# jiaqianjing/kubedl

Hardware: AMD Instinct MI355X
Metric: Job launch delay (s) + steps/sec, PyTorchJob ResNet-50 at 1/2/4/8 MI355X (higher is better)
Workload: dtype bf16

## Files before the change

csrc/bindings.cpp:

```cpp
#include <map>
#include <mutex>
#include <cstring>
#include <torch/extension.h>
#include <ATen/hip/HIPContext.h>
#include <ATen/hip/impl/HIPGuardImplMasqueradingAsCUDA.h>
#include <ATen/hip/impl/HIPStreamMasqueradingAsCUDA.h>

#include "bn_fin.h"
#include "kdl_api.h"

namespace {

int dtype_code(const at::Tensor& t) {
  if (t.scalar_type() == at::kBFloat16) return 1;
  if (t.scalar_type() == at::kFloat) return 0;
  TORCH_CHECK(false, "kubedl_amd: unsupported dtype ", t.scalar_type());
  return -1;
}

hipStream_t cur_stream() { return c10::hip::getCurrentHIPStreamMasqueradingAsCUDA().stream(); }

void check_hip(hipError_t e, const char* what) {
  TORCH_CHECK(e == hipSuccess, "kubedl_amd: ", what, " failed: ", hipGetErrorString(e));
}
// ... 1363 lines not shown
  const int64_t rows_in = stride > 1 ? (M / (Hout * Wout)) * Hin * Win : M;
  need_bf16(G, M * N, "conv1x1_wgrad G");
  need_bf16(A, rows_in * K, "conv1x1_wgrad A");
  need_opt_f32(pro_coef, 2 * K, "pro_coef");
  const int64_t slabs =
      kdl::conv1x1_wgrad_splits(static_cast<int>(M), static_cast<int>(N), static_cast<int>(K), solo);
  TORCH_CHECK(dw32.is_cuda() && dw32.scalar_type() == at::kFloat && dw32.is_contiguous() &&
                  dw32.numel() >= slabs * N * K,
              "conv1x1_wgrad: dw32 must be fp32 contiguous with conv1x1_wgrad_splits(M, N, K) * N * K elements");
  if (dW.has_value() && dW->defined())
    TORCH_CHECK(dW->is_cuda() && dW->is_contiguous() && dW->numel() == N * K && dW->scalar_type() == at::kBFloat16,
                "conv1x1_wgrad: dW bf16 contiguous [N, K]");
  const c10::hip::HIPGuardMasqueradingAsCUDA guard(G.device());
  check_hip(kdl::conv1x1_wgrad(G.data_ptr(), A.data_ptr(), opt_fptr(pro_coef), dw32.data_ptr<float>(),
                               dW.has_value() && dW->defined() ? dW->data_ptr() : nullptr, static_cast<float>(scale),
                               static_cast<int>(M), static_cast<int>(N), static_cast<int>(K), static_cast<int>(Hout),
                               static_cast<int>(Wout), static_cast<int>(Hin), static_cast<int>(Win),
                               static_cast<int>(stride), cur_stream(), bw.x, bw.coef, solo),
            "conv1x1_wgrad");
}

int64_t conv1x1_gram_floats(int64_t M, int64_t K) {
  return static_cast<int64_t>(kdl::conv1x1_gram_splits(static_cast<int>(M), static_cast<int>(K))) * (K * K + K);
}

void conv1x1_gram(const at::Tensor& X, const at::Tensor& pro, at::Tensor ws, int64_t M, int64_t K) {
  need_bf16(X, M * K, "conv1x1_gram X");
  need_opt_f32(pro, 2 * K, "conv1x1_gram pro");
  need_opt_f32(ws, conv1x1_gram_floats(M, K), "conv1x1_gram ws");
  const c10::hip::HIPGuardMasqueradingAsCUDA guard(X.device());
  check_hip(kdl::conv1x1_gram(X.data_ptr(), pro.data_ptr<float>(), ws.data_ptr<float>(), static_cast<int>(M),
                              static_cast<int>(K), cur_stream()),
            "conv1x1_gram");
}

void gram_fold(const at::Tensor& Gm, const at::Tensor& QS, const at::Tensor& W, const at::Tensor& bcoef, at::Tensor out,
               int64_t N, int64_t K) {
  need_opt_f32(Gm, N * K, "gram_fold G");
  need_opt_f32(QS, K * K + K, "gram_fold Q|s");
  need_opt_f32(bcoef, 3 * N, "gram_fold bcoef");
  need_bf16(W, N * K, "gram_fold W");
  need_bf16(out, N * K, "gram_fold out");
  const c10::hip::HIPGuardMasqueradingAsCUDA guard(W.device());
  check_hip(kdl::gram_fold(Gm.data_ptr<float>(), QS.data_ptr<float>(), W.data_ptr(), bcoef.data_ptr<float>(),
                           static_cast<int>(N), static_cast<int>(K), out.data_ptr(), cur_stream()),
            "gram_fold");
}

void slab_reduce_f32(at::Tensor slabs, int64_t nk, int64_t nsplit) {
  TORCH_CHECK(nk % 4 == 0 && nsplit >= 1, "slab_reduce_f32: nk % 4 == 0");
  need_opt_f32(slabs, nk * nsplit, "slab_reduce_f32 slabs");
  const c10::hip::HIPGuardMasqueradingAsCUDA guard(slabs.device());
  check_hip(kdl::wgrad_slab_reduce(slabs.data_ptr<float>(), nk, static_cast<int>(nsplit), 1.0f, nullptr,
                                   cur_stream()),
            "slab_reduce_f32");
}

void conv3x3_wgrad(const at::Tensor& G, const at::Tensor& A, const c10::optional<at::Tensor>& pro_coef,
                   at::Tensor dw32, const c10::optional<at::Tensor>& dW, double scale, int64_t Nb, int64_t H,
                   int64_t Wd, int64_t Cin, int64_t Cout, int64_t stride) {
  TORCH_CHECK(Cin % 64 == 0 && Cout % 64 == 0 && Nb > 0 && stride >= 1, "conv3x3_wgrad: need Cin, Cout % 64 == 0");
  const int64_t Ho = (H - 1) / stride + 1, Wo = (Wd - 1) / stride + 1, M = Nb * Ho * Wo, K = 9 * Cin;
  need_bf16(G, M * Cout, "conv3x3_wgrad G");
  need_bf16(A, Nb * H * Wd * Cin, "conv3x3_wgrad A");
  need_opt_f32(pro_coef, 2 * Cin, "pro_coef");
  const int64_t slabs = kdl::conv1x1_wgrad_splits(static_cast<int>(M), static_cast<int>(Cout), static_cast<int>(K));
// ... 245 lines not shown
  m.def("gemm_dgrad_relu", &gemm_dgrad_relu, "(dz W) * [y > 0] and its column sums (bf16): data gradient through a ReLU + bias gradient, one launch");
  m.def("relu_bwd_dbias", &relu_bwd_dbias, "ReLU backward (mask from output) + bias gradient (deterministic; bf16 or fp32)",
        py::arg("dy"), py::arg("y"), py::arg("db_bf16") = false);
  m.def("head_bce_fwd", &head_bce_fwd, "1-wide logit layer + sigmoid BCE: (logit, dlogit, per-block loss sums)");
  m.def("head_bce_bwd", &head_bce_bwd,
        "logit layer backward: (dx, dw, db, per-block dw partials, per-block db partials[, dbx: relu_x])",
        py::arg("x"), py::arg("w"), py::arg("dlogit"), py::arg("scale"), py::arg("gscale"), py::arg("relu_x") = false);
  m.def("embed_gather", &embed_gather, "embedding row gather into a [B, ld] activation");
  m.def("segment_reduce", &segment_reduce, "sorted segment sum of gradient rows", py::arg("rows"), py::arg("F"),
        py::arg("col0"), py::arg("D"), py::arg("order"), py::arg("seg"), py::arg("ucount") = py::none(),
        py::arg("out_rows") = py::none(), py::arg("out") = py::none());
  m.def("a2a_route", &a2a_route, "fixed-capacity exchange: per-owner send blocks + header + rslot of unique ids");
  m.def("a2a_owner_update", &a2a_owner_update, "owner Adagrad update of a fixed exchange without de-duplication",
        py::arg("grads"), py::arg("local"), py::arg("cap"), py::arg("W"), py::arg("slotmap"), py::arg("call"),
        py::arg("table"), py::arg("accum"), py::arg("lr"), py::arg("eps"), py::arg("scale"),
        py::arg("stamped") = false);
  m.def("a2a_serve", &a2a_serve, "owner side of the fixed exchange: requested rows + local row ids (+ the owner "
        "update's slot stamps)",
        py::arg("table"), py::arg("req"), py::arg("n_own"), py::arg("rows_bf16") = false,
        py::arg("slotmap") = py::none(), py::arg("call") = 0, py::arg("cap") = 0, py::arg("W") = 0);
  m.def("embed_gather_cast", &embed_gather_cast,
        "fused one-owner pull: bf16(table[uniq[inv]]) into the tower input (+ tail: dense columns, zero pad)",
        py::arg("table"), py::arg("uniq"), py::arg("inv"), py::arg("F"), py::arg("out"), py::arg("col0"),
        py::arg("dense") = py::none(), py::arg("tail") = 0);
  m.def("segment_adagrad", &segment_adagrad, "segment sum + fused sparse Adagrad on owned rows");
  m.def("dedup_table_slots", &dedup_table_slots, "hash-table slots dedup_csr needs for n ids");
  m.def("segment_reduce_adagrad", &segment_reduce_adagrad,
        "one-owner sync-free push: per-id gradient sums (segment_reduce) applied by Adagrad in the same launch");
  m.def("csr_from_inverse_only", &csr_from_inverse_only, "CSR (seg, order) of a dedup_csr inverse, positions ascending per id");
  m.def("dedup_csr", &dedup_csr, "sync-free id de-duplication (uniq/inv/count on the device) + optional CSR of the inverse");
  m.def("conv1x1_gemm", &conv1x1_gemm, "1x1 conv / dgrad as MFMA GEMM with fused BN prologue/epilogue");
  m.def("set_stem_drop", &kdl::set_stem_drop, "timing-only: skip the stem kernel's MFMAs (1), epilogue (2), input (4)");
  m.def("conv1x1_gram_floats", &conv1x1_gram_floats, "workspace floats of conv1x1_gram(M, K)");
  m.def("conv1x1_gram", &conv1x1_gram, "Q = a^T a | s = 1^T a of a = relu(X*scale+shift) (fp32, into ws[:K*K+K])");
  m.def("gram_fold", &gram_fold, "dW = diag(k) G + diag(c1) W Q + c0 s^T -> bf16 (BN-backward weight gradient, dc never stored)");
  m.def("slab_reduce_f32", &slab_reduce_f32, "fixed-order fp32 sum of slabs into the first");
  m.def("bn_bwd_pro_arm", &bn_bwd_pro_arm, "fuse this BN's backward apply (input x, workspace ws) into the next conv1x1_gemm's A (or conv1x1_wgrad's G) staging; optional write-through tensor");
  m.def("bn_fin_arm", &bn_fin_arm, "fold the BN finalize of this workspace (C channels, M elements) into the next conv GEMM launch");
  m.def("bn_fin_desc", &bn_fin_desc, "write a BN layer's finalize descriptor into its workspace tail");
  m.def("stem7x7_wgrad_bn", &stem7x7_wgrad_bn, "stem weight gradient with the stem BN+ReLU+max-pool backward folded in");
  m.def("stem7x7_wgrad", &stem7x7_wgrad, "ResNet stem 7x7/s2/p3 conv weight gradient -> [64][224] bf16 (stem K order)");
  m.def("stem7x7_wgrad_slabs", [](int64_t nb, int64_t h, int64_t w) {
          return kdl::stem7x7_wgrad_slabs(static_cast<int>(nb), static_cast<int>(h), static_cast<int>(w)); },
        "fp32 slab count of stem7x7_wgrad's workspace", py::arg("nb"), py::arg("h") = 224, py::arg("w") = 224);
  m.def("head_splits", &head_splits, "K splits (fc forward, dfeat) of the classifier head kernels");
  m.def("head_lpad", [](int64_t L) { return kdl::head_lpad(static_cast<int>(L)); }, "row pitch of the head's dl");
  m.def("head_forward", &head_forward, "classifier head forward: mean pool + fc (MFMA) + softmax CE + dlogits");
  m.def("head_backward", &head_backward, "classifier head backward: dfeat, dW, db (MFMA) + mean loss");
  m.def("stem7x7_fwd", &stem7x7_fwd, "ResNet stem 7x7/s2/p3 conv (224 -> 112, 3 -> 64 channels) with BN statistics epilogue");
  m.def("conv3x3_s2_dgrad", &conv3x3_s2_dgrad,
        "stride-2 3x3 pad-1 conv data gradient: four sub-pixel class GEMMs, PLAIN or MASKX epilogue",
        py::arg("dy"), py::arg("ball"), py::arg("dx"), py::arg("Nb"), py::arg("Hd"), py::arg("Wd"), py::arg("Cd"),
        py::arg("N"), py::arg("epi"), py::arg("acc"), py::arg("ex"), py::arg("emean"), py::arg("ecoef"),
        py::arg("Hx") = 0, py::arg("Wx") = 0);
  m.def("bn_res_pro_arm", &bn_res_pro_arm, "next forward conv1x1_gemm applies relu(A*scale+shift+res), written through + mask");
  m.def("conv3x3_aout_arm", &conv3x3_aout_arm, "next prologue conv3x3_gemm also writes relu(B(x)) here (56x56 halo)");
  m.def("conv3x3_gemm", &conv3x3_gemm, "3x3 pad-1 conv (fwd or stride-1 dgrad) as implicit MFMA GEMM with fused BN prologue/epilogue");
  m.def("conv1x1_wgrad", &conv1x1_wgrad, "1x1 conv weight gradient (split-M MFMA into fp32 slabs, fixed-order reduce + bf16 cast); solo: no side stream shares the GPU (more splits)",
        py::arg("G"), py::arg("A"), py::arg("pro_coef"), py::arg("dw32"), py::arg("dW"), py::arg("scale"), py::arg("M"),
        py::arg("N"), py::arg("K"), py::arg("Hout"), py::arg("Wout"), py::arg("Hin"), py::arg("Win"), py::arg("stride"),
        py::arg("solo") = false);
  m.def("conv3x3_wgrad", &conv3x3_wgrad, "3x3 pad-1 conv weight gradient (implicit GEMM, split-M slabs)");
  m.def("conv3x3_wgrad_slabs", &conv3x3_wgrad_slabs, "fp32 [Cout, 9 Cin] slabs conv3x3_wgrad may write (its fastest path)");
  m.def("set_wgrad_big", &kdl::set_wgrad_big, "256x256 weight-gradient tiles: 0 off, 1 3x3 only, 2 3x3 + 1x1");
  m.def("conv1x1_wgrad_splits", &conv1x1_wgrad_splits, "M splits (slab count) of conv1x1_wgrad", py::arg("M"),
        py::arg("N"), py::arg("K"), py::arg("solo") = false);
// ... 12 lines not shown
```

csrc/conv1x1.hip:

```cpp
#include <cstdlib>
#include <type_traits>

#include "common.h"
#include "gemm_epi.h"
#include "kdl_api.h"
#include "tune.h"

namespace kdl {
namespace {

using namespace gemm;

constexpr int kThreads = 256;
constexpr int BK = 64;
__host__ __device__ constexpr int bwd_kmax(int bn) { return bn >= 128 ? 512 : 2048; }

enum { PRO_NONE = 0, PRO_FWD = 1, PRO_BWD = 2, PRO_RES = 5, PRO_RES2 = 6 };

template <int BM, int BN, int MINB, int PRO, int GATHER, int EPI, int KBK = BK>
__global__ __launch_bounds__(kThreads, MINB) void gemm1x1_kernel(GemmParams p, int GM, int tiles_m, int tiles_n) {
  static_assert((PRO != PRO_BWD && PRO != PRO_RES && PRO != PRO_RES2) || GATHER == G_DENSE,
                "the two-input prologues read dense rows");
  constexpr bool TWO_IN = PRO == PRO_BWD || PRO == PRO_RES || PRO == PRO_RES2;
  constexpr int LDK = KBK + 8;
// ... 723 lines not shown
  const int a = wgrad_splits(M, N, K, false), b = wgrad_splits(M, N, K, false, true);
  const int c = solo ? wgrad_splits(M, N, K, false, false, true) : 0;
  return a > b ? (a > c ? a : c) : (b > c ? b : c);
}

void set_wgrad_big(int mode) {
  static const bool env = tune_has("wgrad_big");
  if (!env) g_wgrad_big = mode;
}

namespace {
template <int TN_, int TK_>
void launch_wgrad(dim3 grid, hipStream_t s, const bf16_t* g, const bf16_t* x, const float* pro, float* dw32, int M,
                  int N, int K, int Hout, int Wout, int Hin, int Win, int stride, int rps, int tiles_k, int mode,
                  int cin) {
#define WG_LAUNCH(P, G)                                                                                             \
  hipLaunchKernelGGL((wgrad1x1_kernel<TN_, TK_, P, G>), grid, dim3(kThreads), 0, s, g, x, pro, dw32, M, N, K, Hout, \
                     Wout, Hin, Win, stride, rps, tiles_k, cin)
  if (pro) {
    if (mode == G_CONV3) WG_LAUNCH(true, G_CONV3);
    else if (mode == G_STRIDED) WG_LAUNCH(true, G_STRIDED);
    else WG_LAUNCH(true, G_DENSE);
  } else {
    if (mode == G_CONV3) WG_LAUNCH(false, G_CONV3);
    else if (mode == G_STRIDED) WG_LAUNCH(false, G_STRIDED);
    else WG_LAUNCH(false, G_DENSE);
  }
#undef WG_LAUNCH
}
}

namespace {
hipError_t wgrad_reduce(float* dw32, int64_t nk, int nsplit, float scale, bf16_t* dW, hipStream_t s,
                        int layout = 0) {
  static const bool skip = tune_int("price_wgrad_reduce", 1) == 0;
  if (skip) return hipSuccess;
  const int rgrid = static_cast<int>((nk / 4 + kRedCols - 1) / kRedCols);
  static const int red_target = tune_int("wgrad_red_blocks", 2048);
  int groups = (red_target + rgrid - 1) / rgrid;
  const int by_work = (nsplit + 31) / 32;
  if (groups > by_work) groups = by_work;
  if (groups <= 1) {
    hipLaunchKernelGGL(wgrad_reduce_kernel, dim3(rgrid), dim3(kThreads), 0, s, dw32, nk, nsplit, nsplit, 1, scale,
                       dW, layout);
    return hipGetLastError();
  }
  const int chunk = (nsplit + groups - 1) / groups;
  groups = (nsplit + chunk - 1) / chunk;
  hipLaunchKernelGGL(wgrad_reduce_kernel, dim3(rgrid, groups), dim3(kThreads), 0, s, dw32, nk, nsplit, chunk, 1,
                     1.0f, static_cast<bf16_t*>(nullptr), 0);
  hipLaunchKernelGGL(wgrad_reduce_kernel, dim3(rgrid), dim3(kThreads), 0, s, dw32, nk, groups, groups, chunk, scale,
                     dW, layout);
  return hipGetLastError();
}

constexpr int kFoldJ = 16;
__global__ __launch_bounds__(256) void gram_fold_kernel(const float* __restrict__ Gm, const float* __restrict__ QS,
                                                        const bf16_t* __restrict__ W, const float* __restrict__ bcoef,
                                                        int N, int K, bf16_t* __restrict__ out) {
  __shared__ float Ws[kFoldJ][64 + 4];
  __shared__ __attribute__((aligned(16))) float Qs[kFoldJ][64];
  const int n0 = blockIdx.y * 64, k0 = blockIdx.x * 64;
  const int t = threadIdx.x, tn = (t >> 4) * 4, tk = (t & 15) * 4;
  float acc[4][4];
#pragma unroll
  for (int i = 0; i < 4; ++i)
#pragma unroll
    for (int q = 0; q < 4; ++q) acc[i][q] = 0.f;
  const int wr = t >> 2, wc = (t & 3) * 4;
  const int qr = t >> 4, qc = (t & 15) * 4;
  for (int j0 = 0; j0 < K; j0 += kFoldJ) {
    const bf16_t* w = W + static_cast<int64_t>(n0 + wr) * K + j0 + wc;
// ... 235 lines not shown
    wp.a_rows = mode == G_DENSE ? M : static_cast<int64_t>(M / (Hout * Wout)) * Hin * Win;
    if (mode != G_DENSE) {
      wp.mg_hw = static_cast<uint32_t>(((uint64_t(1) << 32) + Hout * Wout - 1) / (Hout * Wout));
      wp.mg_w = static_cast<uint32_t>(((uint64_t(1) << 32) + Wout - 1) / Wout);
    }
    const hipError_t e = wgrad_dma(wp, nsplit, tn, tk, s);
    if (e != hipSuccess && e != hipErrorInvalidValue) return e;
    done = e == hipSuccess;
  }
  if (!done && bwd) return hipErrorInvalidValue;
  if (!done) {
    if (tn > 128 || tk > 128) {
      tn = tk = 128;
      tiles_k = K / tk;
      grid = dim3(nsplit * (N / tn) * tiles_k);
    }
    if (tn == 128 && tk == 128) launch_wgrad<128, 128>(grid, s, g, x, pro_coef, dw32, M, N, K, Hout, Wout, Hin, Win, stride, rps, tiles_k, mode, cin);
    else if (tn == 128) launch_wgrad<128, 64>(grid, s, g, x, pro_coef, dw32, M, N, K, Hout, Wout, Hin, Win, stride, rps, tiles_k, mode, cin);
    else if (tk == 128) launch_wgrad<64, 128>(grid, s, g, x, pro_coef, dw32, M, N, K, Hout, Wout, Hin, Win, stride, rps, tiles_k, mode, cin);
    else launch_wgrad<64, 64>(grid, s, g, x, pro_coef, dw32, M, N, K, Hout, Wout, Hin, Win, stride, rps, tiles_k, mode, cin);
    RETURN_IF_HIP_ERR(hipGetLastError());
  }
  return wgrad_reduce(dw32, static_cast<int64_t>(N) * K, nsplit, scale, static_cast<bf16_t*>(dW), s);
}
}

hipError_t conv1x1_wgrad(const void* G, const void* A, const float* pro_coef, float* dw32, void* dW, float scale,
                         int M, int N, int K, int Hout, int Wout, int Hin, int Win, int stride, hipStream_t s,
                         const void* gx, const float* gcoef, bool solo) {
  return wgrad_impl(G, A, pro_coef, dw32, dW, scale, M, N, K, Hout, Wout, Hin, Win, stride,
                    stride > 1 ? G_STRIDED : G_DENSE, K, s, false, gx, gcoef, solo);
}

int conv3x3_wgrad_slabs(int Nb, int Hin, int Win, int Cin, int Cout, int stride) {
  const int Ho = (Hin - 1) / stride + 1, Wo = (Win - 1) / stride + 1;
  const int M = Nb * Ho * Wo;
  const int a = conv1x1_wgrad_splits(M, Cout, 9 * Cin), b = wgrad_splits(M, Cout, 9 * Cin, true);
  const int dflt = a > b ? a : b;
  const int halo = halo3x3_wgrad_slabs(Nb, Hin, Win, Cin, Cout, stride);
  return halo > dflt ? halo : dflt;
}

hipError_t conv3x3_wgrad(const void* G, const void* A, const float* pro_coef, float* dw32, int64_t dw32_floats,
                         void* dW, float scale, int Nb, int Hin, int Win, int Cin, int Cout, int stride,
                         hipStream_t s) {
  if (Cin % 64 || Cout % 64 || Nb <= 0 || stride < 1) return hipErrorInvalidValue;
  if (gemm_core_mode() != 0) {
    int nslabs = 0;
    const hipError_t e = halo3x3_wgrad(G, A, pro_coef, dw32, dw32_floats, Nb, Hin, Win, Cin, Cout, stride, &nslabs, s);
    if (e == hipSuccess)
      return wgrad_reduce(dw32, static_cast<int64_t>(Cout) * 9 * Cin, nslabs, scale, static_cast<bf16_t*>(dW), s);
    if (e != hipErrorInvalidValue) return e;
  }
  const int Ho = (Hin - 1) / stride + 1, Wo = (Win - 1) / stride + 1;
  const int M = Nb * Ho * Wo;
  const bool big = dw32_floats >= static_cast<int64_t>(wgrad_splits(M, Cout, 9 * Cin, true)) * Cout * 9 * Cin;
  return wgrad_impl(G, A, pro_coef, dw32, dW, scale, M, Cout, 9 * Cin, Ho, Wo, Hin, Win, stride, G_CONV3, Cin, s,
                    big);
}

}
```

csrc/gemm_epi.h:

```cpp
#pragma once

#include "bn_fin.h"
#include "common.h"

namespace kdl {
namespace gemm {

typedef __attribute__((ext_vector_type(8))) __bf16 bf16x8_t;
typedef __attribute__((ext_vector_type(16))) float f32x16_t;
typedef __attribute__((ext_vector_type(4))) float f32x4_t;
typedef __attribute__((ext_vector_type(2))) float f2_t;

constexpr int kRep = 32;

enum { EPI_PLAIN = 0, EPI_STATS = 1, EPI_MASKX = 2, EPI_RESBITS = 3, EPI_RES = 4, EPI_BIAS = 5, EPI_BIAS_RELU = 6 };
enum { G_DENSE = 0, G_STRIDED = 1, G_CONV3 = 2, G_DGRAD2 = 3, G_STEM = 4 };

struct GemmParams {
  const bf16_t* A;
  const bf16_t* B;
  bf16_t* C;
  int M, N, K;
  int Hout, Wout, Hin, Win, stride;
  int Cin;
// ... 4 lines not shown
  const float* bcoef2;
  bf16_t* aout;
  const float* shift;
  const bf16_t* bias16;
  float* acc;
  const bf16_t* ex;
  const float* emean;
  const float* ecoef;
  const bf16_t* eres;
  int res_stride;
  int res_H, res_W;
  const uint8_t* ebits;
  const bf16_t* ex2;
  const float* emean2;
  float* acc2;
  int price_drop;
  int mc, mc_pad;
  float* fin_ws;
  float* fin_ws2;
  float fin_M;
  uint8_t* obits;
};

struct WgParams {
  const bf16_t* G;
  const bf16_t* A;
  const float* pro;
  const bf16_t* gx;
  const float* gcoef;
  float* dw32;
  int M, N, K;
  int Hout, Wout, Hin, Win, stride, cin;
  int rps, tiles_k, mode;
  int64_t a_rows;
  uint32_t mg_hw, mg_w;
};
hipError_t wgrad_dma(const WgParams& p, int nsplit, int tn, int tk, hipStream_t s);

int igemm_pick(int M, int N, int K);
bool g_forced_cfg_unset();
hipError_t igemm(const GemmParams& p, int epi, int gather, int cfg, hipStream_t s);
hipError_t halo3x3(const GemmParams& p, int epi, hipStream_t s);
int halo3x3_wgrad_slabs(int Nb, int Hin, int Win, int Cin, int Cout, int stride);
hipError_t halo3x3_wgrad(const void* G, const void* A, const float* pro, float* dw32, int64_t dw32_floats, int Nb,
                         int Hin, int Win, int Cin, int Cout, int stride, int* nslabs, hipStream_t s);

__device__ __forceinline__ uint4 ld16(const bf16_t* p) { return *reinterpret_cast<const uint4*>(p); }

__device__ __forceinline__ void unpack8(const uint4 v, float (&o)[8]) {
  const uint32_t w[4] = {v.x, v.y, v.z, v.w};
#pragma unroll
  for (int i = 0; i < 4; ++i) {
    o[2 * i] = __uint_as_float(w[i] << 16);
    o[2 * i + 1] = __uint_as_float(w[i] & 0xffff0000u);
  }
}

__device__ __forceinline__ void unpack4x2(const uint4 v, f2_t (&o)[4]) {
  const uint32_t w[4] = {v.x, v.y, v.z, v.w};
#pragma unroll
  for (int i = 0; i < 4; ++i) o[i] = f2_t{__uint_as_float(w[i] << 16), __uint_as_float(w[i] & 0xffff0000u)};
}

__device__ __forceinline__ uint32_t pack2(const f2_t v) { return pack_bf16x2(v.x, v.y); }

__device__ __forceinline__ f2_t pfma(const f2_t a, const f2_t b, const f2_t c) {
// ... 329 lines not shown
```

csrc/kdl_api.h:

```cpp
#pragma once

#include <hip/hip_runtime.h>
#include <stdint.h>

namespace kdl {

int64_t bn_workspace_floats(int C);
hipError_t bn_act_forward(const void* x, const void* res, void* y, uint8_t* mbits, const void* gamma,
                          const void* beta, float* rm, float* rv, float* save_mean,
                          float* save_invstd, float* ws, int64_t M, int C, int dtype, int pdtype,
                          bool relu, bool training, float momentum, float eps, hipStream_t s);
hipError_t bn_act_backward(const void* dy, const void* y, const uint8_t* mbits, const void* x,
                           const void* gamma,
                           const void* beta, const float* mean, const float* invstd, void* dx,
                           void* dres, void* dgamma, void* dbeta, float* ws, int64_t M, int C,
                           int dtype, int pdtype, bool relu, bool training, hipStream_t s);

hipError_t bn_pool_forward(const void* x, void* y, uint8_t* idx, const void* gamma, const void* beta,
                           float* rm, float* rv, float* save_mean, float* save_invstd, float* ws,
                           int N, int H, int W, int C, int pdtype, bool training, float momentum,
                           float eps, hipStream_t s,
                           bool gemm_stats = false, void* xam = nullptr);
hipError_t bn_pool_backward(const void* dyp, const uint8_t* idx, const void* x, const void* gamma,
                            const void* beta, const float* mean, const float* invstd, void* dx,
// ... 221 lines not shown
  const void* ex2;
  const float* emean2;
  float* acc2;
  int ksize;
  int Cin;
  float* fin_ws;
  float* fin_ws2;
  float fin_M;
  const void* bx;
  const float* bcoef;
  const float* bcoef2;
  void* aout;
  int bres;
  uint8_t* obits;
};
hipError_t conv1x1_gemm(const Conv1x1Args& a, hipStream_t s);
hipError_t conv3x3_dgrad_s2(const Conv1x1Args& a, hipStream_t s);
hipError_t stem7x7_fwd(const void* x, const void* wp, void* y, int Nb, int H, int W, const float* shift, float* acc,
                       hipStream_t s, bool raw_w = false);
int stem7x7_wgrad_slabs(int Nb, int H = 224, int W = 224);
hipError_t stem7x7_wgrad(const void* dy, const void* x, float* dw32, void* dW, int Nb, int H, int W, hipStream_t s,
                         bool raw_out = false);
hipError_t stem7x7_wgrad_bn(const void* c0, const void* dp, const uint8_t* idx, const float* coef5, const void* x,
                            float* dw32, void* dW, int Nb, hipStream_t s, bool raw_out = false);
void head_splits(int Nb, int C, int L, int* s1, int* s2);
int head_lpad(int L);
hipError_t head_forward(const void* x, int Nb, int HW, int C, const void* w, const void* b, int L, const int64_t* y,
                        void* feat, float* part1, float* lrow, void* dl, void* dlT, hipStream_t s);
hipError_t head_backward(const void* feat, const void* w, const void* dl, const void* dlT, int Nb, int C, int L,
                         float* part2, void* dfeat, void* dW, void* db, const float* lrow, float* loss,
                         hipStream_t s);
int conv1x1_gram_splits(int M, int K);
hipError_t conv1x1_gram(const void* X, const float* pro, float* ws, int M, int K, hipStream_t s);
hipError_t gram_fold(const float* Gm, const float* QS, const void* W, const float* bcoef, int N, int K, void* out,
                     hipStream_t s);
hipError_t wgrad_slab_reduce(float* dw32, int64_t nk, int nsplit, float scale, void* dW, hipStream_t s,
                             int layout = 0);
void set_stem_drop(int bits);
int conv1x1_wgrad_splits(int M, int N, int K, bool solo = false);
void set_wgrad_big(int mode);
hipError_t conv1x1_wgrad(const void* G, const void* A, const float* pro_coef, float* dw32, void* dW, float scale,
                         int M, int N, int K, int Hout, int Wout, int Hin, int Win, int stride, hipStream_t s,
                         const void* gx = nullptr, const float* gcoef = nullptr, bool solo = false);
int conv3x3_wgrad_slabs(int Nb, int Hin, int Win, int Cin, int Cout, int stride);
hipError_t conv3x3_wgrad(const void* G, const void* A, const float* pro_coef, float* dw32, int64_t dw32_floats,
                         void* dW, float scale, int Nb, int Hin, int Win, int Cin, int Cout, int stride,
                         hipStream_t s);

hipError_t cast_copy(const void* src, int sdtype, void* dst, int ddtype, int64_t n, hipStream_t s);

hipError_t make_stream(bool dedicated, int priority, hipStream_t* out, int cus = 0);
hipError_t spin(hipStream_t s, double microseconds);

int gemm_core_mode();
void set_gemm_core_mode(int m);
void set_igemm_cfg(int cfg);
void set_halo3x3(int on);

}
```

csrc/wgrad_dma.hip:

```cpp
#include "common.h"
#include "gemm_epi.h"
#include "kdl_api.h"
#include "lds_dma.h"

#include <type_traits>

namespace kdl {
namespace gemm {
namespace {

using lds_dma::dma16;
using lds_dma::i32x4_t;
using lds_dma::kOOB;
using lds_dma::lds_void_t;
using lds_dma::publish_stage;
using lds_dma::rsrc_words;
typedef short v4s_t __attribute__((ext_vector_type(4)));
typedef __attribute__((address_space(3))) v4s_t lds_v4s_t;

constexpr int MK = 64;

__device__ __forceinline__ v4s_t tr_read(const char* p) {
#if defined(__HIP_DEVICE_COMPILE__)
  return __builtin_amdgcn_ds_read_tr16_b64_v4i16((lds_v4s_t*)(p));
#else
  return v4s_t{};
#endif
}

__device__ __forceinline__ bf16x8_t frag8(v4s_t lo, v4s_t hi) {
  const uint2 a = __builtin_bit_cast(uint2, lo), b = __builtin_bit_cast(uint2, hi);
  return __builtin_bit_cast(bf16x8_t, make_uint4(a.x, a.y, b.x, b.y));
}

template <int TN_, int TK_, int GATHER, bool PRO, int WN = 2, int WK = 2, bool BWDG = false>
__global__ __launch_bounds__(64 * WN * WK, (WN * WK == 4) ? 2 : 1) void wgrad_dma_kernel(WgParams p) {
  constexpr int NW = WN * WK;
  constexpr int PN = TN_ / 64, PK = TK_ / 64;
  constexpr int PX = BWDG ? PN : 0;
  constexpr int PANEL = MK * 128;
  constexpr int STAGE = (PN + PK + PX) * PANEL;
  static_assert((PN + PK + PX) * (MK / 8) % NW == 0, "every wave issues the same DMA count");
  constexpr int IPW = (PN + PK + PX) * (MK / 8) / NW;
  constexpr int TN = TN_ / WN / 32, TK = TK_ / WK / 32;
  static_assert(TN >= 1 && TK >= 1, "wave tile = whole 32x32 MFMA blocks");
  __shared__ __attribute__((aligned(1024))) char lds[2 * STAGE];

  const int t = threadIdx.x, lane = t & 63;
  const int wave = __builtin_amdgcn_readfirstlane(t >> 6);
  const int nblk = gridDim.x, bid = blockIdx.x;
  const int xq = nblk >> 3, xr = nblk & 7, xcd = bid & 7;
  const int wid = (xcd < xr ? xcd * (xq + 1) : xr * (xq + 1) + (xcd - xr) * xq) + (bid >> 3);
  const int tiles = (p.N / TN_) * p.tiles_k;
  const int split = wid / tiles, tile = wid - split * tiles;
  const int tn = tile / p.tiles_k, tk = tile - tn * p.tiles_k;
  const int n0 = tn * TN_, k0 = tk * TK_;
  const int mbeg = split * p.rps;
  const int mend = min(p.M, mbeg + p.rps);
  const int tap = GATHER == G_CONV3 ? k0 / p.cin : 0;
  const int kin0 = k0 - tap * p.cin;
  const int tr3 = tap / 3, tq3 = tap - 3 * (tap / 3);
  const int lda = GATHER == G_CONV3 ? p.cin : p.K;
  const int acol0 = GATHER == G_CONV3 ? kin0 : k0;

  const i32x4_t wG = rsrc_words(p.G, static_cast<uint32_t>(static_cast<int64_t>(p.M) * p.N * 2));
  const i32x4_t wA = rsrc_words(p.A, static_cast<uint32_t>(p.a_rows * lda * 2));
  const i32x4_t wX = rsrc_words(BWDG ? p.gx : p.G, static_cast<uint32_t>(static_cast<int64_t>(p.M) * p.N * 2));

  const int lrow = lane >> 3;
// ... 40 lines not shown
    }
  };
  const int grp = lane >> 4, q = (lane & 15) >> 2, pp = lane & 3;
  const int swz = ((q >> 1) & 1) * 4;
  const int rowb = (8 * (grp >> 1) + q) * 128;
  auto frag_off = [&](int col32) {
    const int chunk = (col32 + 16 * (grp & 1) + 4 * pp) >> 3;
    return rowb + 16 * (chunk ^ swz) + 8 * (pp & 1);
  };
  const int wn0 = (wave / WK) * (TN_ / WN), wk0 = (wave % WK) * (TK_ / WK);
  int goff[TN], aoff[TK];
#pragma unroll
  for (int i = 0; i < TN; ++i) {
    const int n = wn0 + 32 * i;
    goff[i] = (n / 64) * PANEL + frag_off(n % 64);
  }
#pragma unroll
  for (int j = 0; j < TK; ++j) {
    const int k = wk0 + 32 * j;
    aoff[j] = (PN + k / 64) * PANEL + frag_off(k % 64);
  }
  float psc[TK], psf[TK];
#pragma unroll
  for (int j = 0; j < TK; ++j) {
    psc[j] = 1.f;
    psf[j] = 0.f;
    if constexpr (PRO) {
      const int kc = acol0 + wk0 + 32 * j + (lane & 31);
      psc[j] = p.pro[kc];
      psf[j] = p.pro[lda + kc];
    }
  }
  (void)psc; (void)psf;
  float gk[TN], gc1[TN], gc0[TN];
#pragma unroll
  for (int i = 0; i < TN; ++i) {
    gk[i] = 1.f;
    gc1[i] = 0.f;
    gc0[i] = 0.f;
    if constexpr (BWDG) {
      const int n = n0 + wn0 + 32 * i + (lane & 31);
      gk[i] = p.gcoef[n];
      gc1[i] = p.gcoef[p.N + n];
      gc0[i] = p.gcoef[2 * p.N + n];
    }
  }
  (void)gk; (void)gc1; (void)gc0;

  f32x16_t acc[TN][TK];
#pragma unroll
  for (int i = 0; i < TN; ++i)
#pragma unroll
    for (int j = 0; j < TK; ++j) acc[i][j] = f32x16_t{};

  constexpr int NMF = 4 * TN * TK;
  constexpr int SPAN = NMF < 2 * IPW ? 1 : (NMF / 2 > IPW ? NMF / 2 : IPW);
  auto raw = [&](const char* S, int s, bf16x8_t (&gf)[TN], bf16x8_t (&xf)[TN], bf16x8_t (&af)[TK]) {
#pragma unroll
    for (int i = 0; i < TN; ++i) {
      const char* b = S + goff[i] + s * 16 * 128;
      gf[i] = frag8(tr_read(b), tr_read(b + 4 * 128));
      if constexpr (BWDG) {
        const char* bx = b + (PN + PK) * PANEL;
        xf[i] = frag8(tr_read(bx), tr_read(bx + 4 * 128));
      }
    }
#pragma unroll
    for (int j = 0; j < TK; ++j) {
      const char* b = S + aoff[j] + s * 16 * 128;
      af[j] = frag8(tr_read(b), tr_read(b + 4 * 128));
    }
  };
  auto prologue = [&](int m0, int s, bool tail, bf16x8_t (&gf)[TN], const bf16x8_t (&xf)[TN], bf16x8_t (&af)[TK]) {
    (void)m0; (void)s; (void)tail; (void)gf; (void)xf; (void)af;
    const int mrow = m0 + 16 * s + 8 * (lane >> 5);
    (void)mrow;
    if constexpr (BWDG) {
#pragma unroll
      for (int i = 0; i < TN; ++i) {
        float f[8], x[8];
        unpack8(__builtin_bit_cast(uint4, gf[i]), f);
        unpack8(__builtin_bit_cast(uint4, xf[i]), x);
#pragma unroll
        for (int e = 0; e < 8; ++e) {
          const float o = fmaf(gk[i], f[e], fmaf(gc1[i], x[e], gc0[i]));
          f[e] = (!tail || mrow + e < mend) ? o : 0.f;
        }
        gf[i] = __builtin_bit_cast(bf16x8_t, pack8(f));
      }
    }
    if constexpr (PRO) {
#pragma unroll
      for (int j = 0; j < TK; ++j) {
        float f[8];
        unpack8(__builtin_bit_cast(uint4, af[j]), f);
#pragma unroll
        for (int e = 0; e < 8; ++e) {
          const float o = fmaf(f[e], psc[j], psf[j]);
          f[e] = (o > 0.f && (!tail || mrow + e < mend)) ? o : 0.f;
        }
        af[j] = __builtin_bit_cast(bf16x8_t, pack8(f));
      }
    }
  };
  auto step = [&](const char* S, int m0, auto issue_tag, int next_stage) {
    constexpr bool ISSUE = decltype(issue_tag)::value;
    const bool tail = (PRO || BWDG) && m0 + MK > mend;
    bf16x8_t gf[2][TN], xf[2][TN], af[2][TK];
    raw(S, 0, gf[0], xf[0], af[0]);
#pragma unroll
    for (int s = 0; s < 4; ++s) {
      prologue(m0, s, tail, gf[s & 1], xf[s & 1], af[s & 1]);
      if (s < 3) raw(S, s + 1, gf[(s + 1) & 1], xf[(s + 1) & 1], af[(s + 1) & 1]);
      __builtin_amdgcn_sched_barrier(0);
#pragma unroll
      for (int i = 0; i < TN; ++i)
#pragma unroll
        for (int j = 0; j < TK; ++j) {
          const int mi = (s * TN + i) * TK + j;
          if constexpr (ISSUE && SPAN == 1) {
            if (mi == 0) {
#pragma unroll
              for (int pi = 0; pi < IPW; ++pi) piece(pi, m0 + MK, next_stage);
            }
          }
          acc[i][j] = __builtin_amdgcn_mfma_f32_32x32x16_bf16(gf[s & 1][i], af[s & 1][j], acc[i][j], 0, 0, 0);
          if constexpr (ISSUE && SPAN > 1) {
#pragma unroll
            for (int pi = 0; pi < IPW; ++pi)
              if (pi * SPAN / IPW == mi) piece(pi, m0 + MK, next_stage);
          }
        }
    }
  };
  using yes = std::integral_constant<bool, true>;
  using no = std::integral_constant<bool, false>;
  if (mbeg < mend) {
#pragma unroll
    for (int i = 0; i < IPW; ++i) piece(i, mbeg, 0);
    int st = 0, m0 = mbeg;
    for (; m0 + MK < mend; m0 += MK) {
      publish_stage();
      step(lds + st * STAGE, m0, yes{}, st ^ 1);
      st ^= 1;
    }
    publish_stage();
    step(lds + st * STAGE, m0, no{}, 0);
  }
  float* slab = p.dw32 + static_cast<int64_t>(split) * p.N * p.K;
  const int fr = lane & 31, fh = lane >> 5;
#pragma unroll
  for (int i = 0; i < TN; ++i)
#pragma unroll
    for (int j = 0; j < TK; ++j)
#pragma unroll
      for (int r = 0; r < 16; ++r) {
        const int n = n0 + wn0 + i * 32 + (r & 3) + 8 * (r >> 2) + 4 * fh;
        const int k = k0 + wk0 + j * 32 + fr;
        slab_store(slab + static_cast<int64_t>(n) * p.K + k, acc[i][j][r]);
      }
}

template <int TN_, int TK_, int WN = 2, int WK = 2>
void launch(const WgParams& p, int grid, hipStream_t s) {
#define WGD_LAUNCH(G, P) \
  hipLaunchKernelGGL((wgrad_dma_kernel<TN_, TK_, G, P, WN, WK>), dim3(grid), dim3(64 * WN * WK), 0, s, p)
  if (p.pro) {
    if (p.mode == G_CONV3) WGD_LAUNCH(G_CONV3, true);
    else if (p.mode == G_STRIDED) WGD_LAUNCH(G_STRIDED, true);
    else WGD_LAUNCH(G_DENSE, true);
  } else {
    if (p.mode == G_CONV3) WGD_LAUNCH(G_CONV3, false);
    else if (p.mode == G_STRIDED) WGD_LAUNCH(G_STRIDED, false);
    else WGD_LAUNCH(G_DENSE, false);
  }
#undef WGD_LAUNCH
}

template <int TN_, int TK_, int WN, int WK>
void launch_bwdg(const WgParams& p, int grid, hipStream_t s) {
#define WGD_LAUNCH_B(G, P) \
  hipLaunchKernelGGL((wgrad_dma_kernel<TN_, TK_, G, P, WN, WK, true>), dim3(grid), dim3(64 * WN * WK), 0, s, p)
  if (p.mode == G_STRIDED) WGD_LAUNCH_B(G_STRIDED, false);
  else if (p.pro) WGD_LAUNCH_B(G_DENSE, true);
  else WGD_LAUNCH_B(G_DENSE, false);
#undef WGD_LAUNCH_B
}

}

hipError_t wgrad_dma(const WgParams& p, int nsplit, int tn, int tk, hipStream_t s) {
  const int lda = p.mode == G_CONV3 ? p.cin : p.K;
  if ((p.pro && p.mode == G_CONV3) || p.rps % MK || p.N % tn || p.K % tk || (p.mode == G_CONV3 && p.cin % tk) ||
      static_cast<int64_t>(p.M) * p.N * 2 >= (int64_t(1) << 31) || p.a_rows * lda * 2 >= (int64_t(1) << 31))
    return hipErrorInvalidValue;
  if (p.mode != G_DENSE &&
      static_cast<uint64_t>(p.M) * static_cast<uint64_t>(p.Hout * p.Wout) >= (uint64_t(1) << 32))
    return hipErrorInvalidValue;
  const int grid = nsplit * (p.N / tn) * (p.K / tk);
  if (p.gx) {
    if (!p.gcoef || p.mode == G_CONV3 || (p.pro && p.mode != G_DENSE)) return hipErrorInvalidValue;
    if (tn == 128 && tk == 256) launch_bwdg<128, 256, 2, 4>(p, grid, s);
    else if (tn == 128 && tk == 128) launch_bwdg<128, 128, 2, 4>(p, grid, s);
    else if (tn == 128 && tk == 64) launch_bwdg<128, 64, 4, 2>(p, grid, s);
    else if (tn == 64 && tk == 256) launch_bwdg<64, 256, 2, 4>(p, grid, s);
    else if (tn == 64 && tk == 128) launch_bwdg<64, 128, 2, 4>(p, grid, s);
    else if (tn == 64 && tk == 64) launch_bwdg<64, 64, 2, 2>(p, grid, s);
    else return hipErrorInvalidValue;
    return hipGetLastError();
  }
  if (tn == 256 && tk == 256) launch<256, 256, 2, 4>(p, grid, s);
  else if (tn == 128 && tk == 128) launch<128, 128>(p, grid, s);
  else if (tn == 128) launch<128, 64>(p, grid, s);
  else if (tk == 128) launch<64, 128>(p, grid, s);
  else launch<64, 64>(p, grid, s);
  return hipGetLastError();
}

}
}
```

kubedl_amd/models/resnet_engine.py:

```python
from __future__ import annotations

import contextlib
import math
import dataclasses
import os

import torch
import torch.nn.functional as F

from kubedl_amd.models.resnet import BNAct, Bottleneck, ResNet
from kubedl_amd.ops.conv import S2_TAPS, s2_dgrad_weights, stem_grad_from_k, stem_weights

REP = 32


def _nhwc_empty(n, c, h, w, like):
    return torch.empty((n, c, h, w), dtype=like.dtype, device=like.device, memory_format=torch.channels_last)


def _rows(t: torch.Tensor) -> torch.Tensor:
    n, c, h, w = t.shape
    return t.permute(0, 2, 3, 1).reshape(n * h * w, c)


# ... 247 lines not shown
        if prev is None:
            self._arm_bpro(bpro, cout)
            self.ext.conv1x1_gemm(g, wt, out, M, cin, cout, 0, 0, 0, 0, 1, None, 4, None, None, None, None, None, eres,
                                  res_stride, h, w, None, None, None, None)
        else:
            mbits, c3, st3, cd, std_ = prev
            self._arm(st3, M, std_, fwd=False)
            self._arm_bpro(bpro, cout)
            self.ext.conv1x1_gemm(g, wt, out, M, cin, cout, 0, 0, 0, 0, 1, None, 3, None, self._bwd_acc(st3), c3,
                                  st3.save_mean, None, eres, res_stride, h, w, mbits, cd,
                                  std_.save_mean if std_ is not None else None,
                                  self._bwd_acc(std_) if std_ is not None else None)
        return out

    def wgrad(self, g, x, stride, pro: BNState | None, dW, gbpro=None):
        n, cout, ho, wo = g.shape
        _, cin, h, w = x.shape
        M = n * ho * wo
        key = (M, cout, cin)
        need = self.ext.conv1x1_wgrad_splits(M, cout, cin) * cout * cin
        dw32 = self._dw32.get(key)
        if dw32 is None or dw32.numel() < need:
            dw32 = self._dw32[key] = torch.empty(need, device=g.device)
        if gbpro is not None:
            self.ext.bn_bwd_pro_arm(gbpro[0], gbpro[1].ws, cout, None)
        self.ext.conv1x1_wgrad(g, x, self.fcoef(pro) if pro is not None else None, dw32, dW.view(cout, cin), 1.0,
                               M, cout, cin, ho, wo, h, w, stride)

    def wgrad_gram(self, g, x2, st2: BNState | None, st3: BNState, w3, dW):
        n, cout, ho, wo = g.shape
        _, cin, h, w = x2.shape
        M = n * ho * wo
        key = (M, cout, cin)
        need = self.ext.conv1x1_wgrad_splits(M, cout, cin) * cout * cin
        dw32 = self._dw32.get(key)
        if dw32 is None or dw32.numel() < need:
            dw32 = self._dw32[key] = torch.empty(need, device=g.device)
        pro = self.fcoef(st2) if st2 is not None else None
        self.ext.conv1x1_wgrad(g, x2, pro, dw32, None, 1.0, M, cout, cin, ho, wo, h, w, 1)
        if pro is None:
            pro = self._ident.get(cin)
            if pro is None:
                pro = self._ident[cin] = torch.cat([torch.ones(cin, device=g.device), torch.zeros(cin, device=g.device)])
        qs = self._ws32(("gram", M, cin), self.ext.conv1x1_gram_floats(M, cin))
        self.ext.conv1x1_gram(x2, pro, qs, M, cin)
        self.ext.gram_fold(dw32, qs, w3.view(cout, cin), self.bcoef(st3), dW.view(cout, cin), cout, cin)

    def wgrad3x3(self, g, x, stride, dW, pro: BNState | None = None):
        n, cout, ho, wo = g.shape
        _, cin, h, w = x.shape
        M = n * ho * wo
        key = (M, cout, 9 * cin, h, stride)
        need = self.ext.conv3x3_wgrad_slabs(n, h, w, cin, cout, stride) * cout * 9 * cin
        dw32 = self._dw32.get(key)
        if dw32 is None or dw32.numel() < need:
            dw32 = self._dw32[key] = torch.empty(need, device=g.device)
        self.ext.conv3x3_wgrad(g, x, self.fcoef(pro) if pro is not None else None, dw32, dW, 1.0, n, h, w, cin, cout,
                               stride)

    def stem_wgrad(self, dc0, x, dw):
        ws = self._stem_ws(x.shape[0], x.device, x.shape[2], x.shape[3])
        if dw.is_contiguous(memory_format=torch.channels_last):
            self.ext.stem7x7_wgrad(dc0, x, ws[0], dw)
        else:
            self.ext.stem7x7_wgrad(dc0, x, ws[0], ws[1])
            dw.copy_(stem_grad_from_k(ws[1]))

    def stem_bwd(self, dp, idx, c0, st, dgamma, dbeta, with_dx=True):
        m = st.mod
        dx, dg, db = self.ext.bn_pool_bwd(dp, idx, c0, m.weight, m.bias, st.save_mean, st.save_invstd, True, st.ws,
                                          with_dx)
# ... 687 lines not shown
```

Measured before the change: 13920.

## Fuse Gram matrix and column sums into the 1x1 weight-gradient kernel

Adds a GRAM variant of the DMA weight-gradient kernel that also accumulates a^T a (via extra MFMAs on the already-staged A fragments) and column sums of a, written into per-split slabs after G^T a. The wgrad_gram path in the engine then uses one launch plus a reduction instead of a separate wgrad launch and a separate conv1x1_gram pass that re-reads X. This removes one full read of the activation and one kernel launch per bottleneck. In exchange it adds register pressure and extra MFMA and store work to the wgrad kernel, enlarges the workspace, and only applies when K is 64 or 128, falling back otherwise.

```diff
diff --git a/csrc/bindings.cpp b/csrc/bindings.cpp
--- a/csrc/bindings.cpp
+++ b/csrc/bindings.cpp
@@ -1419,6 +1419,26 @@
   check_hip(kdl::conv1x1_gram(X.data_ptr(), pro.data_ptr<float>(), ws.data_ptr<float>(), static_cast<int>(M),
                               static_cast<int>(K), cur_stream()),
             "conv1x1_gram");
+}
+
+int64_t conv1x1_wgrad_gram_floats(int64_t M, int64_t N, int64_t K) {
+  return kdl::conv1x1_wgrad_gram_floats(static_cast<int>(M), static_cast<int>(N), static_cast<int>(K));
+}
+
+bool conv1x1_wgrad_gram(const at::Tensor& G, const at::Tensor& A, const c10::optional<at::Tensor>& pro, at::Tensor ws,
+                        int64_t M, int64_t N, int64_t K) {
+  TORCH_CHECK(K % 64 == 0 && N % 64 == 0 && M > 0, "conv1x1_wgrad_gram: need K % 64 == 0, N % 64 == 0");
+  need_bf16(G, M * N, "conv1x1_wgrad_gram G");
+  need_bf16(A, M * K, "conv1x1_wgrad_gram A");
+  need_opt_f32(pro, 2 * K, "conv1x1_wgrad_gram pro");
+  need_opt_f32(ws, conv1x1_wgrad_gram_floats(M, N, K), "conv1x1_wgrad_gram ws");
+  const c10::hip::HIPGuardMasqueradingAsCUDA guard(G.device());
+  const hipError_t e = kdl::conv1x1_wgrad_gram(G.data_ptr(), A.data_ptr(), opt_fptr(pro), ws.data_ptr<float>(),
+                                               static_cast<int>(M), static_cast<int>(N), static_cast<int>(K),
+                                               cur_stream());
+  if (e == hipErrorInvalidValue) return false;
+  check_hip(e, "conv1x1_wgrad_gram");
+  return true;
 }
 
 void gram_fold(const at::Tensor& Gm, const at::Tensor& QS, const at::Tensor& W, const at::Tensor& bcoef, at::Tensor out,
@@ -1730,6 +1750,9 @@
   m.def("conv1x1_gemm", &conv1x1_gemm, "1x1 conv / dgrad as MFMA GEMM with fused BN prologue/epilogue");
   m.def("set_stem_drop", &kdl::set_stem_drop, "timing-only: skip the stem kernel's MFMAs (1), epilogue (2), input (4)");
   m.def("conv1x1_gram_floats", &conv1x1_gram_floats, "workspace floats of conv1x1_gram(M, K)");
+  m.def("conv1x1_wgrad_gram_floats", &conv1x1_wgrad_gram_floats, "workspace floats of conv1x1_wgrad_gram(M, N, K)");
+  m.def("conv1x1_wgrad_gram", &conv1x1_wgrad_gram,
+        "G^T a | a^T a | 1^T a (fp32, into ws[:N*K + K*K + K]) from one weight-gradient launch; false = not covered");
   m.def("conv1x1_gram", &conv1x1_gram, "Q = a^T a | s = 1^T a of a = relu(X*scale+shift) (fp32, into ws[:K*K+K])");
   m.def("gram_fold", &gram_fold, "dW = diag(k) G + diag(c1) W Q + c0 s^T -> bf16 (BN-backward weight gradient, dc never stored)");
   m.def("slab_reduce_f32", &slab_reduce_f32, "fixed-order fp32 sum of slabs into the first");
diff --git a/csrc/conv1x1.hip b/csrc/conv1x1.hip
--- a/csrc/conv1x1.hip
+++ b/csrc/conv1x1.hip
@@ -779,12 +779,13 @@
 
 namespace {
 hipError_t wgrad_reduce(float* dw32, int64_t nk, int nsplit, float scale, bf16_t* dW, hipStream_t s,
-                        int layout = 0) {
+                        int layout = 0, int64_t group_nk = 0) {
   static const bool skip = tune_int("price_wgrad_reduce", 1) == 0;
   if (skip) return hipSuccess;
   const int rgrid = static_cast<int>((nk / 4 + kRedCols - 1) / kRedCols);
   static const int red_target = tune_int("wgrad_red_blocks", 2048);
-  int groups = (red_target + rgrid - 1) / rgrid;
+  const int ggrid = group_nk ? static_cast<int>((group_nk / 4 + kRedCols - 1) / kRedCols) : rgrid;
+  int groups = (red_target + ggrid - 1) / ggrid;
   const int by_work = (nsplit + 31) / 32;
   if (groups > by_work) groups = by_work;
   if (groups <= 1) {
@@ -1086,6 +1087,30 @@
                     stride > 1 ? G_STRIDED : G_DENSE, K, s, false, gx, gcoef, solo);
 }
 
+int64_t conv1x1_wgrad_gram_floats(int M, int N, int K) {
+  return wgrad_splits(M, N, K, false) * (static_cast<int64_t>(N) * K + static_cast<int64_t>(K) * K + K);
+}
+
+hipError_t conv1x1_wgrad_gram(const void* G, const void* A, const float* pro, float* ws, int M, int N, int K,
+                              hipStream_t s) {
+  if (tune_int("wgrad_gram_fused", 1) == 0 || gemm_core_mode() == 0) return hipErrorInvalidValue;
+  if (M <= 0 || N % 64 || (K != 64 && K != 128)) return hipErrorInvalidValue;
+  int tn, tk;
+  wgrad_tiles(N, K, false, &tn, &tk);
+  const int splits = wgrad_splits(M, N, K, false);
+  int rps = (M + splits - 1) / splits;
+  rps = (rps + WMK - 1) / WMK * WMK;
+  const int nsplit = (M + rps - 1) / rps;
+  WgParams wp{};
+  wp.G = static_cast<const bf16_t*>(G); wp.A = static_cast<const bf16_t*>(A); wp.pro = pro; wp.dw32 = ws;
+  wp.M = M; wp.N = N; wp.K = K; wp.stride = 1; wp.cin = K; wp.rps = rps; wp.tiles_k = K / tk; wp.mode = G_DENSE;
+  wp.a_rows = M;
+  wp.gram = 1;
+  RETURN_IF_HIP_ERR(wgrad_dma(wp, nsplit, tn, tk, s));
+  const int64_t gnk = static_cast<int64_t>(N) * K;
+  return wgrad_reduce(ws, gnk + static_cast<int64_t>(K) * K + K, nsplit, 1.f, nullptr, s, 0, gnk);
+}
+
 int conv3x3_wgrad_slabs(int Nb, int Hin, int Win, int Cin, int Cout, int stride) {
   const int Ho = (Hin - 1) / stride + 1, Wo = (Win - 1) / stride + 1;
   const int M = Nb * Ho * Wo;
diff --git a/csrc/gemm_epi.h b/csrc/gemm_epi.h
--- a/csrc/gemm_epi.h
+++ b/csrc/gemm_epi.h
@@ -60,6 +60,7 @@
   int M, N, K;
   int Hout, Wout, Hin, Win, stride, cin;
   int rps, tiles_k, mode;
+  int gram;
   int64_t a_rows;
   uint32_t mg_hw, mg_w;
 };
diff --git a/csrc/kdl_api.h b/csrc/kdl_api.h
--- a/csrc/kdl_api.h
+++ b/csrc/kdl_api.h
@@ -277,6 +277,9 @@
                          hipStream_t s);
 int conv1x1_gram_splits(int M, int K);
 hipError_t conv1x1_gram(const void* X, const float* pro, float* ws, int M, int K, hipStream_t s);
+int64_t conv1x1_wgrad_gram_floats(int M, int N, int K);
+hipError_t conv1x1_wgrad_gram(const void* G, const void* A, const float* pro, float* ws, int M, int N, int K,
+                              hipStream_t s);
 hipError_t gram_fold(const float* Gm, const float* QS, const void* W, const float* bcoef, int N, int K, void* out,
                      hipStream_t s);
 hipError_t wgrad_slab_reduce(float* dw32, int64_t nk, int nsplit, float scale, void* dW, hipStream_t s,
diff --git a/csrc/wgrad_dma.hip b/csrc/wgrad_dma.hip
--- a/csrc/wgrad_dma.hip
+++ b/csrc/wgrad_dma.hip
@@ -33,8 +33,10 @@
   return __builtin_bit_cast(bf16x8_t, make_uint4(a.x, a.y, b.x, b.y));
 }
 
-template <int TN_, int TK_, int GATHER, bool PRO, int WN = 2, int WK = 2, bool BWDG = false>
+template <int TN_, int TK_, int GATHER, bool PRO, int WN = 2, int WK = 2, bool BWDG = false, bool GRAM = false>
 __global__ __launch_bounds__(64 * WN * WK, (WN * WK == 4) ? 2 : 1) void wgrad_dma_kernel(WgParams p) {
+  static_assert(!GRAM || (GATHER == G_DENSE && !BWDG && WN == 2 && WK == 2 && TN_ == 128 && (TK_ == 64 || TK_ == 128)),
+                "GRAM: dense 1x1, 2 x 2 waves, tiles 128 x 64 / 128 x 128");
   constexpr int NW = WN * WK;
   constexpr int PN = TN_ / 64, PK = TK_ / 64;
   constexpr int PX = BWDG ? PN : 0;
@@ -141,6 +143,28 @@
     }
   }
   (void)psc; (void)psf;
+  const int wq_n = wave / WK, wq_k = wave % WK;
+  const bool has_q = GRAM && tn < TK_ / 32 && (TK == 2 || wq_n == 0);
+  const bool has_s = GRAM && tn == 0 && wq_n == 0;
+  const int qrb = tn, qj = TK == 2 ? wq_n : 0, qcb = wq_k * TK + qj;
+  const bool qread = has_q && qrb != qcb;
+  int qoff = 0;
+  float qsc = 1.f, qsf = 0.f;
+  if constexpr (GRAM) {
+    if (has_q) {
+      qoff = (PN + (32 * qrb) / 64) * PANEL + frag_off((32 * qrb) % 64);
+      if constexpr (PRO) {
+        qsc = p.pro[32 * qrb + (lane & 31)];
+        qsf = p.pro[lda + 32 * qrb + (lane & 31)];
+      }
+    }
+  }
+  (void)has_q; (void)has_s; (void)qj; (void)qcb; (void)qread; (void)qoff; (void)qsc; (void)qsf;
+  f32x16_t qacc = f32x16_t{};
+  float csum[TK];
+#pragma unroll
+  for (int j = 0; j < TK; ++j) csum[j] = 0.f;
+  (void)qacc; (void)csum;
   float gk[TN], gc1[TN], gc0[TN];
 #pragma unroll
   for (int i = 0; i < TN; ++i) {
@@ -180,6 +204,24 @@
       af[j] = frag8(tr_read(b), tr_read(b + 4 * 128));
     }
   };
+  auto rawq = [&](const char* S, int s, bf16x8_t& qf) {
+    if constexpr (GRAM) {
+      if (qread) {
+        const char* b = S + qoff + s * 16 * 128;
+        qf = frag8(tr_read(b), tr_read(b + 4 * 128));
+      }
+    }
+  };
+  auto pro_frag = [&](bf16x8_t& a, float sc, float sf, bool tail, int mrow) {
+    float f[8];
+    unpack8(__builtin_bit_cast(uint4, a), f);
+#pragma unroll
+    for (int e = 0; e < 8; ++e) {
+      const float o = fmaf(f[e], sc, sf);
+      f[e] = (o > 0.f && (!tail || mrow + e < mend)) ? o : 0.f;
+    }
+    a = __builtin_bit_cast(bf16x8_t, pack8(f));
+  };
   auto prologue = [&](int m0, int s, bool tail, bf16x8_t (&gf)[TN], const bf16x8_t (&xf)[TN], bf16x8_t (&af)[TK]) {
     (void)m0; (void)s; (void)tail; (void)gf; (void)xf; (void)af;
     const int mrow = m0 + 16 * s + 8 * (lane >> 5);
@@ -200,27 +242,28 @@
     }
     if constexpr (PRO) {
 #pragma unroll
-      for (int j = 0; j < TK; ++j) {
-        float f[8];
-        unpack8(__builtin_bit_cast(uint4, af[j]), f);
-#pragma unroll
-        for (int e = 0; e < 8; ++e) {
-          const float o = fmaf(f[e], psc[j], psf[j]);
-          f[e] = (o > 0.f && (!tail || mrow + e < mend)) ? o : 0.f;
-        }
-        af[j] = __builtin_bit_cast(bf16x8_t, pack8(f));
-      }
+      for (int j = 0; j < TK; ++j) pro_frag(af[j], psc[j], psf[j], tail, mrow);
+    }
+  };
+  auto prologue_q = [&](int m0, int s, bool tail, bf16x8_t& qf) {
+    if constexpr (GRAM && PRO) {
+      if (qread) pro_frag(qf, qsc, qsf, tail, m0 + 16 * s + 8 * (lane >> 5));
     }
   };
   auto step = [&](const char* S, int m0, auto issue_tag, int next_stage) {
     constexpr bool ISSUE = decltype(issue_tag)::value;
     const bool tail = (PRO || BWDG) && m0 + MK > mend;
-    bf16x8_t gf[2][TN], xf[2][TN], af[2][TK];
+    bf16x8_t gf[2][TN], xf[2][TN], af[2][TK], qf[2] = {};
     raw(S, 0, gf[0], xf[0], af[0]);
+    rawq(S, 0, qf[0]);
 #pragma unroll
     for (int s = 0; s < 4; ++s) {
       prologue(m0, s, tail, gf[s & 1], xf[s & 1], af[s & 1]);
-      if (s < 3) raw(S, s + 1, gf[(s + 1) & 1], xf[(s + 1) & 1], af[(s + 1) & 1]);
+      prologue_q(m0, s, tail, qf[s & 1]);
+      if (s < 3) {
+        raw(S, s + 1, gf[(s + 1) & 1], xf[(s + 1) & 1], af[(s + 1) & 1]);
+        rawq(S, s + 1, qf[(s + 1) & 1]);
+      }
       __builtin_amdgcn_sched_barrier(0);
 #pragma unroll
       for (int i = 0; i < TN; ++i)
@@ -240,6 +283,20 @@
               if (pi * SPAN / IPW == mi) piece(pi, m0 + MK, next_stage);
           }
         }
+      if constexpr (GRAM) {
+        if (has_q) {
+          const bf16x8_t ac = (TK == 2 && qj) ? af[s & 1][TK - 1] : af[s & 1][0];
+          qacc = __builtin_amdgcn_mfma_f32_32x32x16_bf16(qread ? qf[s & 1] : ac, ac, qacc, 0, 0, 0);
+        }
+        if (has_s) {
+#pragma unroll
+          for (int j = 0; j < TK; ++j) {
+            float f[8];
+            unpack8(__builtin_bit_cast(uint4, af[s & 1][j]), f);
+            csum[j] += ((f[0] + f[1]) + (f[2] + f[3])) + ((f[4] + f[5]) + (f[6] + f[7]));
+          }
+        }
+      }
     }
   };
   using yes = std::integral_constant<bool, true>;
@@ -256,7 +313,8 @@
     publish_stage();
     step(lds + st * STAGE, m0, no{}, 0);
   }
-  float* slab = p.dw32 + static_cast<int64_t>(split) * p.N * p.K;
+  const int64_t gfloats = static_cast<int64_t>(p.N) * p.K;
+  float* slab = p.dw32 + split * (gfloats + (GRAM ? TK_ * TK_ + TK_ : 0));
   const int fr = lane & 31, fh = lane >> 5;
 #pragma unroll
   for (int i = 0; i < TN; ++i)
@@ -268,6 +326,21 @@
         const int k = k0 + wk0 + j * 32 + fr;
         slab_store(slab + static_cast<int64_t>(n) * p.K + k, acc[i][j][r]);
       }
+  if constexpr (GRAM) {
+    float* qs = slab + gfloats;
+    if (has_q) {
+#pragma unroll
+      for (int r = 0; r < 16; ++r)
+        slab_store(qs + (32 * qrb + (r & 3) + 8 * (r >> 2) + 4 * fh) * TK_ + 32 * qcb + fr, qacc[r]);
+    }
+    if (has_s) {
+#pragma unroll
+      for (int j = 0; j < TK; ++j) {
+        const float v = csum[j] + __shfl_xor(csum[j], 32);
+        if (fh == 0) slab_store(qs + TK_ * TK_ + wk0 + 32 * j + fr, v);
+      }
+    }
+  }
 }
 
 template <int TN_, int TK_, int WN = 2, int WK = 2>
@@ -296,6 +369,14 @@
 #undef WGD_LAUNCH_B
 }
 
+template <int TK_>
+void launch_gram(const WgParams& p, int grid, hipStream_t s) {
+  if (p.pro)
+    hipLaunchKernelGGL((wgrad_dma_kernel<128, TK_, G_DENSE, true, 2, 2, false, true>), dim3(grid), dim3(256), 0, s, p);
+  else
+    hipLaunchKernelGGL((wgrad_dma_kernel<128, TK_, G_DENSE, false, 2, 2, false, true>), dim3(grid), dim3(256), 0, s, p);
+}
+
 }
 
 hipError_t wgrad_dma(const WgParams& p, int nsplit, int tn, int tk, hipStream_t s) {
@@ -307,6 +388,14 @@
       static_cast<uint64_t>(p.M) * static_cast<uint64_t>(p.Hout * p.Wout) >= (uint64_t(1) << 32))
     return hipErrorInvalidValue;
   const int grid = nsplit * (p.N / tn) * (p.K / tk);
+  if (p.gram) {
+    if (p.gx || p.mode != G_DENSE || tn != 128 || (tk != 64 && tk != 128) || p.K != tk || p.tiles_k != 1 ||
+        (p.N / tn) * (tk == 128 ? 4 : 2) < (tk / 32) * (tk / 32))
+      return hipErrorInvalidValue;
+    if (tk == 128) launch_gram<128>(p, grid, s);
+    else launch_gram<64>(p, grid, s);
+    return hipGetLastError();
+  }
   if (p.gx) {
     if (!p.gcoef || p.mode == G_CONV3 || (p.pro && p.mode != G_DENSE)) return hipErrorInvalidValue;
     if (tn == 128 && tk == 256) launch_bwdg<128, 256, 2, 4>(p, grid, s);
diff --git a/kubedl_amd/models/resnet_engine.py b/kubedl_amd/models/resnet_engine.py
--- a/kubedl_amd/models/resnet_engine.py
+++ b/kubedl_amd/models/resnet_engine.py
@@ -303,11 +303,16 @@
         _, cin, h, w = x2.shape
         M = n * ho * wo
         key = (M, cout, cin)
-        need = self.ext.conv1x1_wgrad_splits(M, cout, cin) * cout * cin
+        need = max(self.ext.conv1x1_wgrad_splits(M, cout, cin) * cout * cin,
+                   self.ext.conv1x1_wgrad_gram_floats(M, cout, cin))
         dw32 = self._dw32.get(key)
         if dw32 is None or dw32.numel() < need:
             dw32 = self._dw32[key] = torch.empty(need, device=g.device)
         pro = self.fcoef(st2) if st2 is not None else None
+        if self.ext.conv1x1_wgrad_gram(g, x2, pro, dw32, M, cout, cin):
+            nk = cout * cin
+            self.ext.gram_fold(dw32[:nk], dw32[nk:], w3.view(cout, cin), self.bcoef(st3), dW.view(cout, cin), cout, cin)
+            return
         self.ext.conv1x1_wgrad(g, x2, pro, dw32, None, 1.0, M, cout, cin, ho, wo, h, w, 1)
         if pro is None:
             pro = self._ident.get(cin)
```

Result: no change. 14000 (median of 6 runs) (+0.6%).
